# yellow-binary-tree/MMDuet

Measured on AMD Instinct MI355X. Metric: video frames/sec (stream decode, 1fps 336px), higher is better.
Workload: dtype bf16

## Files before the change

mmduet_amd/csrc/gemm.hip:

```cpp
#include "common.h"
#include <type_traits>

#include "gemm_ring.h"

template <typename T> struct Frag;
template <> struct Frag<bf16_t> { using type = bf16x8_t; static constexpr int KSTEP = 32; };
template <> struct Frag<float> { using type = float; static constexpr int KSTEP = 4; };

template <typename T, int BM, int BN> struct TileCfg {
    static constexpr int BK = 32;
    static constexpr int PAD = sizeof(T) == 2 ? 8 : 1;
    static constexpr int LD = BK + PAD;
    static constexpr int WM = BM / 2, WN = BN / 2;
    static constexpr int TM = WM / 16, TN = WN / 16;
};

template <typename T, int ROWS, int LD>
__device__ __forceinline__ void stage_tile(T* __restrict__ lds, const T* __restrict__ g, long long ld, int r0, int nrows, int k0, int kend,
                                           int vec, int tid) {
    if constexpr (sizeof(T) == 2) {
        for (int i = tid; i < ROWS * 4; i += 256) {
            int r = i >> 2, c = (i & 3) * 8;
            s16x8_t v = {0, 0, 0, 0, 0, 0, 0, 0};
            int gr = r0 + r, gk = k0 + c;
// ... 96 lines not shown
        __syncthreads();
        if constexpr (sizeof(T) == 2) {
            bf16x8_t xf[C::TM], wf[C::TN];
#pragma unroll
            for (int i = 0; i < C::TM; ++i) xf[i] = *reinterpret_cast<const bf16x8_t*>(Xs + (wm + i * 16 + lr) * C::LD + lq * 8);
#pragma unroll
            for (int j = 0; j < C::TN; ++j) wf[j] = *reinterpret_cast<const bf16x8_t*>(Ws + (wn + j * 16 + lr) * C::LD + lq * 8);
#pragma unroll
            for (int i = 0; i < C::TM; ++i)
#pragma unroll
                for (int j = 0; j < C::TN; ++j) acc[i][j] = __builtin_amdgcn_mfma_f32_16x16x32_bf16(wf[j], xf[i], acc[i][j], 0, 0, 0);
        } else {
#pragma unroll
            for (int kk = 0; kk < C::BK; kk += 4) {
                float xf[C::TM], wf[C::TN];
#pragma unroll
                for (int i = 0; i < C::TM; ++i) xf[i] = Xs[(wm + i * 16 + lr) * C::LD + kk + lq];
#pragma unroll
                for (int j = 0; j < C::TN; ++j) wf[j] = Ws[(wn + j * 16 + lr) * C::LD + kk + lq];
#pragma unroll
                for (int i = 0; i < C::TM; ++i)
#pragma unroll
                    for (int j = 0; j < C::TN; ++j) acc[i][j] = __builtin_amdgcn_mfma_f32_16x16x4f32(wf[j], xf[i], acc[i][j], 0, 0, 0);
            }
        }
    }

    if (gridDim.z > 1) {
        float* ws = p.ws + (long long)blockIdx.z * p.M * p.N;
#pragma unroll
        for (int i = 0; i < C::TM; ++i)
#pragma unroll
            for (int j = 0; j < C::TN; ++j) {
                int m = m0 + wm + i * 16 + lr, n = n0 + wn + j * 16 + lq * 4;
                if (m < p.M) {
                    float* y = ws + (long long)m * p.N + n;
                    if (n + 3 < p.N && (p.N & 3) == 0) *reinterpret_cast<f32x4_t*>(y) = acc[i][j];
                    else for (int r = 0; r < 4; ++r) if (n + r < p.N) y[r] = acc[i][j][r];
                }
            }
        return;
    }
#pragma unroll
    for (int i = 0; i < C::TM; ++i) {
        int m = m0 + wm + i * 16 + lr;
        if (p.epi == EPI_SWIGLU) {
#pragma unroll
            for (int j = 0; j < C::TN; j += 2) {
                int n = n0 + wn + j * 16 + lq * 4;
                float g[4] = {acc[i][j][0], acc[i][j][1], acc[i][j][2], acc[i][j][3]};
                float u[4] = {acc[i][j + 1][0], acc[i][j + 1][1], acc[i][j + 1][2], acc[i][j + 1][3]};
                store4_swiglu<T>(p, m, n, g, u);
            }
        } else {
#pragma unroll
            for (int j = 0; j < C::TN; ++j) {
                int n = n0 + wn + j * 16 + lq * 4;
                float v[4] = {acc[i][j][0], acc[i][j][1], acc[i][j][2], acc[i][j][3]};
                store4<T>(p, m, n, v);
            }
        }
    }
}

template <typename T>
__global__ void splitk_reduce_kernel(GemmP p, int splits) {
    long long idx = (long long)blockIdx.x * blockDim.x + threadIdx.x;
    int n4 = (p.N + 3) / 4;
    if (idx >= (long long)p.M * n4) return;
    int m = (int)(idx / n4), n = (int)(idx % n4) * 4;
    if (p.epi == EPI_SWIGLU) {
        if ((n & 16) != 0) return;
        float g[4] = {0, 0, 0, 0}, u[4] = {0, 0, 0, 0};
        for (int s = 0; s < splits; ++s) {
            const float* w = p.ws + ((long long)s * p.M + m) * p.N + n;
            for (int r = 0; r < 4; ++r) { if (n + r < p.N) g[r] += w[r]; if (n + 16 + r < p.N) u[r] += w[16 + r]; }
        }
        store4_swiglu<T>(p, m, n, g, u);
        return;
    }
    float v[4] = {0, 0, 0, 0};
    for (int s = 0; s < splits; ++s) {
        const float* w = p.ws + ((long long)s * p.M + m) * p.N + n;
        for (int r = 0; r < 4; ++r) if (n + r < p.N) v[r] += w[r];
    }
    store4<T>(p, m, n, v);
}

__global__ void pack_w16x32_kernel(const bf16_t* __restrict__ W, long long ldw, int N, int K, bf16_t* __restrict__ out) {
    long long i = (long long)blockIdx.x * blockDim.x + threadIdx.x;
    int KT = K >> 5;
    long long pieces = (long long)(N >> 4) * KT * 64;
    if (i >= pieces) return;
    int lane = (int)(i & 63);
    long long tile = i >> 6;
    int kt = (int)(tile % KT);
    long long nt = tile / KT;
    const bf16_t* src = W + (nt * 16 + (lane & 15)) * ldw + kt * 32 + (lane >> 4) * 8;
    *reinterpret_cast<s16x8_t*>(out + i * 8) = *reinterpret_cast<const s16x8_t*>(src);
}

hipError_t launch_pack_w(const void* W, int64_t ldw, int N, int K, void* out, hipStream_t st) {
    long long pieces = (long long)(N >> 4) * (K >> 5) * 64;
    if (pieces <= 0) return hipSuccess;
    hipLaunchKernelGGL(pack_w16x32_kernel, dim3(cdiv(pieces, 256)), dim3(256), 0, st, (const bf16_t*)W, (long long)ldw, N, K, (bf16_t*)out);
    return hipGetLastError();
}

__global__ __launch_bounds__(256) void quantize_fp8_rows_kernel(bf16_t* __restrict__ W, int K, uint8_t* __restrict__ q8, float* __restrict__ scale) {
    __shared__ float red[4];
    const long long row = blockIdx.x;
    bf16_t* w = W + row * K;
    float amax = 0.f;
    for (int k = threadIdx.x; k < K; k += 256) amax = fmaxf(amax, fabsf(bf2f(w[k])));
    amax = wave_max(amax);
    if ((threadIdx.x & 63) == 0) red[threadIdx.x >> 6] = amax;
    __syncthreads();
    amax = fmaxf(fmaxf(red[0], red[1]), fmaxf(red[2], red[3]));
    const float sc = amax > 0.f ? amax / 448.0f : 1.0f;
    if (threadIdx.x == 0) scale[row] = sc;
    for (int k = threadIdx.x * 2; k < K; k += 512) {
        const float a = bf2f(w[k]) / sc, b = bf2f(w[k + 1]) / sc;
        const int pk = __builtin_amdgcn_cvt_pk_fp8_f32(a, b, 0, false);
        q8[row * K + k] = (uint8_t)(pk & 0xff); q8[row * K + k + 1] = (uint8_t)((pk >> 8) & 0xff);
        const auto back = __builtin_amdgcn_cvt_pk_f32_fp8(pk, false);
        w[k] = f2bf(back[0]); w[k + 1] = f2bf(back[1]);
    }
}
hipError_t launch_quantize_fp8_rows(void* W, int N, int K, uint8_t* q8, float* scale, hipStream_t st) {
    if (N <= 0 || (K & 1)) return N <= 0 ? hipSuccess : hipErrorInvalidValue;
    hipLaunchKernelGGL(quantize_fp8_rows_kernel, dim3(N), dim3(256), 0, st, (bf16_t*)W, K, q8, scale);
    return hipGetLastError();
}
__global__ void pack_w8_kernel(const uint8_t* __restrict__ q8, int N, int K, uint8_t* __restrict__ out) {
    long long i = (long long)blockIdx.x * blockDim.x + threadIdx.x;
    const int KP = K >> 6;
    const long long pieces = (long long)(N >> 4) * KP * 64;
    if (i >= pieces) return;
    const int lane = (int)(i & 63);
    const long long blk = i >> 6;
    const int kp = (int)(blk % KP);
    const long long nt = blk / KP;
    const uint8_t* src = q8 + (nt * 16 + (lane & 15)) * (long long)K + kp * 64 + (lane >> 4) * 8;
    uint2 lo = *reinterpret_cast<const uint2*>(src), hi = *reinterpret_cast<const uint2*>(src + 32);
    *reinterpret_cast<uint4*>(out + i * 16) = uint4{lo.x, lo.y, hi.x, hi.y};
}
hipError_t launch_pack_w8(const uint8_t* q8, int N, int K, void* out, hipStream_t st) {
    const long long pieces = (long long)(N >> 4) * (K >> 6) * 64;
    if (pieces <= 0) return hipSuccess;
    hipLaunchKernelGGL(pack_w8_kernel, dim3(cdiv(pieces, 256)), dim3(256), 0, st, q8, N, K, (uint8_t*)out);
    return hipGetLastError();
}
__device__ __forceinline__ bf16x8_t fp8x8_to_bf16(unsigned lo, unsigned hi) {
    typedef __attribute__((ext_vector_type(2))) __bf16 b2;
    const b2 a = __builtin_amdgcn_cvt_scalef32_pk_bf16_fp8((int)lo, 1.0f, false), b = __builtin_amdgcn_cvt_scalef32_pk_bf16_fp8((int)lo, 1.0f, true);
    const b2 c = __builtin_amdgcn_cvt_scalef32_pk_bf16_fp8((int)hi, 1.0f, false), d = __builtin_amdgcn_cvt_scalef32_pk_bf16_fp8((int)hi, 1.0f, true);
    return bf16x8_t{a[0], a[1], b[0], b[1], c[0], c[1], d[0], d[1]};
}

__device__ __forceinline__ int xs_slot(int ktl, int kq, int r) { return kq * 16 + (r ^ (kq + 4 * (ktl & 1))); }

template <int MT, int NT, bool W8 = false>
__global__ __launch_bounds__(256) void gemm_skinny_kernel(GemmP p, int KT, int kt_per_split) {
    constexpr int KS = 4;
    __shared__ __attribute__((aligned(16))) bf16_t Xs[2][MT * KS * 64 * 8];
    const int tid = threadIdx.x, lane = tid & 63, wave = tid >> 6;
    const int lr = lane & 15, lq = lane >> 4;
    const int ntiles = p.N >> 4;
    const int nt0 = (blockIdx.x * 4 + wave) * NT;
    const int kt_beg = blockIdx.y * kt_per_split;
    const int kt_end = min(KT, kt_beg + kt_per_split);
    const bf16_t* X = (const bf16_t*)p.X;
    const bf16_t* Wp = (const bf16_t*)p.W;

    f32x4_t acc[MT][NT];
#pragma unroll
    for (int i = 0; i < MT; ++i)
#pragma unroll
        for (int j = 0; j < NT; ++j) acc[i][j] = f32x4_t{0, 0, 0, 0};

    bf16x8_t wc[NT][KS], wn[NT][KS];
    s16x8_t xr[MT];

    auto load_w = [&](bf16x8_t (&w)[NT][KS], int kt) {
        if constexpr (W8) {
            const uint8_t* W8p = (const uint8_t*)p.W;
#pragma unroll
            for (int j = 0; j < NT; ++j)
#pragma unroll
                for (int s = 0; s < KS; s += 2) {
                    u32x4_t v = {0, 0, 0, 0};
                    if (nt0 + j < ntiles && kt + s < kt_end)
                        v = __builtin_nontemporal_load(reinterpret_cast<const u32x4_t*>(W8p + (((long long)(nt0 + j) * (KT >> 1) + ((kt + s) >> 1)) * 64 + lane) * 16));
                    w[j][s] = fp8x8_to_bf16(v[0], v[1]); w[j][s + 1] = fp8x8_to_bf16(v[2], v[3]);
                }
            return;
        }
#pragma unroll
        for (int j = 0; j < NT; ++j)
#pragma unroll
            for (int s = 0; s < KS; ++s) {
                s16x8_t v = {0, 0, 0, 0, 0, 0, 0, 0};
                if (nt0 + j < ntiles && kt + s < kt_end)
                    v = __builtin_nontemporal_load(reinterpret_cast<const s16x8_t*>(Wp + (((long long)(nt0 + j) * KT + kt + s) * 64 + lane) * 8));
                w[j][s] = __builtin_bit_cast(bf16x8_t, v);
            }
    };
    auto load_x = [&](int kt) {
#pragma unroll
        for (int j = 0; j < MT; ++j) {
            int i = tid + 256 * j, m = i >> 4, c = i & 15;
            s16x8_t v = {0, 0, 0, 0, 0, 0, 0, 0};
            if (m < p.M && kt + (c >> 2) < kt_end) v = *reinterpret_cast<const s16x8_t*>(X + (long long)m * p.ldx + kt * 32 + c * 8);
            xr[j] = v;
        }
    };
    auto write_x = [&](int buf) {
#pragma unroll
        for (int j = 0; j < MT; ++j) {
            int i = tid + 256 * j, m = i >> 4, c = i & 15;
            int mt = m >> 4, r = m & 15, ktl = c >> 2, kq = c & 3;
            *reinterpret_cast<s16x8_t*>(&Xs[buf][((mt * KS + ktl) * 64 + xs_slot(ktl, kq, r)) * 8]) = xr[j];
        }
    };

    load_w(wc, kt_beg);
    load_x(kt_beg);
    write_x(0);
    __syncthreads();
    int cur = 0;
    for (int kt = kt_beg; kt < kt_end; kt += KS) {
        const bool more = kt + KS < kt_end;
        if (more) { load_w(wn, kt + KS); load_x(kt + KS); }
#pragma unroll
        for (int s = 0; s < KS; ++s) {
            if (kt + s < kt_end) {
#pragma unroll
                for (int i = 0; i < MT; ++i) {
                    bf16x8_t xf = *reinterpret_cast<const bf16x8_t*>(&Xs[cur][((i * KS + s) * 64 + xs_slot(s, lq, lr)) * 8]);
#pragma unroll
                    for (int j = 0; j < NT; ++j) acc[i][j] = __builtin_amdgcn_mfma_f32_16x16x32_bf16(wc[j][s], xf, acc[i][j], 0, 0, 0);
                }
            }
        }
        if (more) write_x(cur ^ 1);
        __syncthreads();
#pragma unroll
        for (int j = 0; j < NT; ++j)
#pragma unroll
            for (int s = 0; s < KS; ++s) wc[j][s] = wn[j][s];
        cur ^= 1;
    }

    if (gridDim.y > 1 || p.slabs) {
        float* ws = p.ws + (long long)blockIdx.y * p.M * p.N;
#pragma unroll
        for (int i = 0; i < MT; ++i)
#pragma unroll
            for (int j = 0; j < NT; ++j) {
                int m = i * 16 + lr, n = (nt0 + j) * 16 + lq * 4;
                if (m < p.M && nt0 + j < ntiles) {
                    f32x4_t v = acc[i][j];
                    if (p.slabs && p.wscale) v *= *reinterpret_cast<const f32x4_t*>(p.wscale + n);
                    *reinterpret_cast<f32x4_t*>(ws + (long long)m * p.N + n) = v;
                }
            }
        return;
    }
#pragma unroll
    for (int i = 0; i < MT; ++i) {
        int m = i * 16 + lr;
        if (p.epi == EPI_SWIGLU) {
            if constexpr (NT >= 2) {
#pragma unroll
                for (int j = 0; j < NT; j += 2) {
                    if (nt0 + j + 1 < ntiles) {
                        int n = (nt0 + j) * 16 + lq * 4;
                        float g[4] = {acc[i][j][0], acc[i][j][1], acc[i][j][2], acc[i][j][3]};
                        float u[4] = {acc[i][j + 1][0], acc[i][j + 1][1], acc[i][j + 1][2], acc[i][j + 1][3]};
                        store4_swiglu<bf16_t>(p, m, n, g, u);
                    }
                }
            }
        } else {
#pragma unroll
            for (int j = 0; j < NT; ++j) {
                if (nt0 + j < ntiles) {
                    int n = (nt0 + j) * 16 + lq * 4;
                    float v[4] = {acc[i][j][0], acc[i][j][1], acc[i][j][2], acc[i][j][3]};
                    store4<bf16_t>(p, m, n, v);
                }
            }
        }
    }
}

__device__ __forceinline__ s16x8_t chain_norm8(const s16x8_t& h, const s16x8_t& g, float inv) {
    s16x8_t o;
#pragma unroll
    for (int e = 0; e < 8; ++e) o[e] = (short)f2bf(bf2f((bf16_t)g[e]) * bf2f(f2bf(bf2f((bf16_t)h[e]) * inv)));
    return o;
}

template <int NT, int U, bool W8 = false, bool CHAIN = false, int WAVES = 4>
__global__ __launch_bounds__(WAVES * 64) void gemm_gemv16_kernel(GemmP p, int KT, GemvChain ch) {
    __shared__ __attribute__((aligned(16))) float red[WAVES - 1][NT][64][4];
    constexpr int XW = 1024;
    __shared__ __attribute__((aligned(16))) bf16_t xs[(CHAIN && WAVES == 4) ? WAVES * GEMV_CHAIN_ROWS * XW : 8];
    const int tid = threadIdx.x, lane = tid & 63, wave = tid >> 6;
    const int lr = lane & 15, lq = lane >> 4;
    const int nt0 = blockIdx.x * NT;
    constexpr int KG = W8 ? 2 : 1;
    const int KTg = KT / KG;
    const int ktb = (KTg + gridDim.y - 1) / gridDim.y;
    const int blk_beg = blockIdx.y * ktb, blk_end = min(KTg, blk_beg + ktb);
    const int ktw = (blk_end - blk_beg + WAVES - 1) / WAVES;
    const int kt_beg = blk_beg + wave * ktw, kt_end = min(blk_end, kt_beg + ktw);
    const bool xn = CHAIN && WAVES == 4 && ch.xn_h != nullptr;
    const bf16_t* xrow = (const bf16_t*)p.X + (long long)lr * p.ldx + lq * 8;
    const bf16_t* xl = xs + (wave * GEMV_CHAIN_ROWS + lr) * XW + lq * 8 - kt_beg * (32 * KG);
    const bool row_ok = lr < p.M;

    f32x4_t acc[NT];
#pragma unroll
    for (int j = 0; j < NT; ++j) acc[j] = f32x4_t{0, 0, 0, 0};

    auto chain_prologue = [&]() {
        const int k0 = kt_beg * (32 * KG), kn = (kt_end - kt_beg) * (32 * KG);
        for (int r = 0; r < p.M; ++r) {
            const f32x4_t q = *reinterpret_cast<const f32x4_t*>(ch.xn_ssq + r * GEMV_SSQ_STRIDE + lane * 4);
            s16x8_t hv[2], gv[2];
#pragma unroll
            for (int ps = 0; ps < 2; ++ps) {
                const int k = ps * 512 + lane * 8;
                hv[ps] = s16x8_t{0, 0, 0, 0, 0, 0, 0, 0}; gv[ps] = hv[ps];
                if (k < kn) {
                    hv[ps] = *reinterpret_cast<const s16x8_t*>((const bf16_t*)ch.xn_h + (long long)r * p.K + k0 + k);
                    gv[ps] = *reinterpret_cast<const s16x8_t*>((const bf16_t*)ch.xn_gamma + k0 + k);
                }
            }
            const float inv = rsqrtf(wave_sum((q[0] + q[1]) + (q[2] + q[3])) / (float)p.K + ch.xn_eps);
#pragma unroll
            for (int ps = 0; ps < 2; ++ps) {
                const int k = ps * 512 + lane * 8;
                if (k < kn) *reinterpret_cast<s16x8_t*>(xs + (wave * GEMV_CHAIN_ROWS + r) * XW + k) = chain_norm8(hv[ps], gv[ps], inv);
            }
        }
    };

    if constexpr (W8) {
        const uint8_t* W8p = (const uint8_t*)p.W;
        const int KP = KT >> 1;
        constexpr int UP = U / 2;
        auto iter = [&](int kp0, auto first) {
            u32x4_t wv[NT][UP]; bf16x8_t x[UP][2];
#pragma unroll
            for (int u = 0; u < UP; ++u) {
                const int kp = kp0 + u;
                s16x8_t x0 = {0, 0, 0, 0, 0, 0, 0, 0}, x1 = x0;
                if (kp < kt_end) {
#pragma unroll
                    for (int j = 0; j < NT; ++j)
                        wv[j][u] = __builtin_nontemporal_load(reinterpret_cast<const u32x4_t*>(W8p + (((long long)(nt0 + j) * KP + kp) * 64 + lane) * 16));
                    if (!xn && row_ok) { x0 = *reinterpret_cast<const s16x8_t*>(xrow + kp * 64); x1 = *reinterpret_cast<const s16x8_t*>(xrow + kp * 64 + 32); }
                } else {
#pragma unroll
                    for (int j = 0; j < NT; ++j) wv[j][u] = u32x4_t{0, 0, 0, 0};
                }
                x[u][0] = __builtin_bit_cast(bf16x8_t, x0); x[u][1] = __builtin_bit_cast(bf16x8_t, x1);
            }
            if constexpr (CHAIN) if (xn) {
                if constexpr (decltype(first)::value) chain_prologue();
#pragma unroll
                for (int u = 0; u < UP; ++u) if (row_ok && kp0 + u < kt_end) {
                    x[u][0] = __builtin_bit_cast(bf16x8_t, *reinterpret_cast<const s16x8_t*>(xl + (kp0 + u) * 64));
                    x[u][1] = __builtin_bit_cast(bf16x8_t, *reinterpret_cast<const s16x8_t*>(xl + (kp0 + u) * 64 + 32));
                }
            }
#pragma unroll
            for (int u = 0; u < UP; ++u)
#pragma unroll
                for (int j = 0; j < NT; ++j) {
                    acc[j] = __builtin_amdgcn_mfma_f32_16x16x32_bf16(fp8x8_to_bf16(wv[j][u][0], wv[j][u][1]), x[u][0], acc[j], 0, 0, 0);
                    acc[j] = __builtin_amdgcn_mfma_f32_16x16x32_bf16(fp8x8_to_bf16(wv[j][u][2], wv[j][u][3]), x[u][1], acc[j], 0, 0, 0);
                }
        };
        if (kt_beg < kt_end) {
            iter(kt_beg, std::true_type{});
            for (int kp0 = kt_beg + UP; kp0 < kt_end; kp0 += UP) iter(kp0, std::false_type{});
        }
    } else {
        const bf16_t* Wp = (const bf16_t*)p.W;
        auto iter = [&](int kt0, auto first) {
            bf16x8_t w[NT][U], x[U];
#pragma unroll
            for (int u = 0; u < U; ++u) {
                const int kt = kt0 + u;
                s16x8_t xv = {0, 0, 0, 0, 0, 0, 0, 0};
                if (kt < kt_end) {
#pragma unroll
                    for (int j = 0; j < NT; ++j)
                        w[j][u] = __builtin_bit_cast(bf16x8_t, __builtin_nontemporal_load(reinterpret_cast<const s16x8_t*>(Wp + (((long long)(nt0 + j) * KT + kt) * 64 + lane) * 8)));
                    if (!xn && row_ok) xv = *reinterpret_cast<const s16x8_t*>(xrow + kt * 32);
                } else {
#pragma unroll
                    for (int j = 0; j < NT; ++j) w[j][u] = __builtin_bit_cast(bf16x8_t, xv);
                }
                x[u] = __builtin_bit_cast(bf16x8_t, xv);
            }
            if constexpr (CHAIN) if (xn) {
                if constexpr (decltype(first)::value) chain_prologue();
#pragma unroll
                for (int u = 0; u < U; ++u) if (row_ok && kt0 + u < kt_end) x[u] = __builtin_bit_cast(bf16x8_t, *reinterpret_cast<const s16x8_t*>(xl + (kt0 + u) * 32));
            }
#pragma unroll
            for (int u = 0; u < U; ++u)
#pragma unroll
                for (int j = 0; j < NT; ++j) acc[j] = __builtin_amdgcn_mfma_f32_16x16x32_bf16(w[j][u], x[u], acc[j], 0, 0, 0);
        };
        if (kt_beg < kt_end) {
            iter(kt_beg, std::true_type{});
            for (int kt0 = kt_beg + U; kt0 < kt_end; kt0 += U) iter(kt0, std::false_type{});
        }
    }
    if (wave > 0) {
#pragma unroll
        for (int j = 0; j < NT; ++j) *reinterpret_cast<f32x4_t*>(&red[wave - 1][j][lane][0]) = acc[j];
    }
    __syncthreads();
    if (wave != 0) return;
#pragma unroll
    for (int j = 0; j < NT; ++j)
#pragma unroll
        for (int w2 = 0; w2 < WAVES - 1; ++w2) acc[j] += *reinterpret_cast<const f32x4_t*>(&red[w2][j][lane][0]);
    const int m = lr;
    if constexpr (CHAIN) if (ch.fin_h) {
#pragma unroll
        for (int j = 0; j < NT; ++j) {
            float ss = 0.f;
            if (m < p.M) {
                f32x4_t v = acc[j];
                if (p.wscale) v *= *reinterpret_cast<const f32x4_t*>(p.wscale + (nt0 + j) * 16 + lq * 4);
                bf16_t* hp = (bf16_t*)ch.fin_h + (long long)m * p.N + (nt0 + j) * 16 + lq * 4;
                const s16x4_t r = *reinterpret_cast<const s16x4_t*>(hp);
                s16x4_t o;
#pragma unroll
                for (int e = 0; e < 4; ++e) {
                    const float hv = bf2f(f2bf(bf2f(f2bf(v[e])) + bf2f((bf16_t)r[e])));
                    ss += hv * hv; o[e] = (short)f2bf(hv);
                }
                *reinterpret_cast<s16x4_t*>(hp) = o;
            }
            ss += __shfl_xor(ss, 16, 64); ss += __shfl_xor(ss, 32, 64);
            if (lq == 0 && m < p.M) ch.fin_ssq[m * GEMV_SSQ_STRIDE + nt0 + j] = ss;
        }
        return;
    }
    if (m >= p.M) return;
    if (p.slabs) {
        float* ws = p.ws + (long long)blockIdx.y * p.M * p.N;
#pragma unroll
        for (int j = 0; j < NT; ++j) {
            f32x4_t v = acc[j];
            if (p.wscale) v *= *reinterpret_cast<const f32x4_t*>(p.wscale + (nt0 + j) * 16 + lq * 4);
            *reinterpret_cast<f32x4_t*>(ws + (long long)m * p.N + (nt0 + j) * 16 + lq * 4) = v;
        }
        return;
    }
    if (p.epi == EPI_SWIGLU) {
        if constexpr (NT >= 2) {
#pragma unroll
            for (int j = 0; j < NT; j += 2) {
                float g[4] = {acc[j][0], acc[j][1], acc[j][2], acc[j][3]};
                float u[4] = {acc[j + 1][0], acc[j + 1][1], acc[j + 1][2], acc[j + 1][3]};
                store4_swiglu<bf16_t>(p, m, (nt0 + j) * 16 + lq * 4, g, u);
            }
        }
    } else {
#pragma unroll
        for (int j = 0; j < NT; ++j) {
            float v[4] = {acc[j][0], acc[j][1], acc[j][2], acc[j][3]};
            store4<bf16_t>(p, m, (nt0 + j) * 16 + lq * 4, v);
        }
    }
}

template <int N_, typename F> __device__ __forceinline__ void stream_static_for(F&& f) {
    if constexpr (N_ > 0) { stream_static_for<N_ - 1>(f); f(std::integral_constant<int, N_ - 1>{}); }
}

template <int MT, int NT, int WK, int KS, int NB, int DBG = 0, int WN = 4>
__global__ __launch_bounds__(64 * WN * WK) void gemm_stream_kernel(GemmP p, int KT, int kt_per_block) {
    constexpr int NWAVE = WN * WK, KSB = WK * KS;
    constexpr int XPIECES = MT * KSB;
    constexpr int XP = DBG == 1 ? 0 : (XPIECES + NWAVE - 1) / NWAVE;
    constexpr int NWL = DBG == 2 ? 0 : NT * KS;
    constexpr int LA = NB - 1;
    constexpr int ISSUE = NWL + XP;
    constexpr int VM_STEP = (LA - 1) * ISSUE;
    constexpr int XSLOT = XPIECES * 512;
    static_assert(VM_STEP <= 63, "vmcnt is a 6-bit counter");
    extern __shared__ __attribute__((aligned(16))) bf16_t lds[];
    const int tid = threadIdx.x, lane = tid & 63, wave = __builtin_amdgcn_readfirstlane(tid >> 6);
    const int lr = lane & 15, lq = lane >> 4;
    const int wn = wave % WN, wk = wave / WN;
    const int ntiles = p.N >> 4;
    const int nt0 = (blockIdx.x * WN + wn) * NT;
    const int kt_beg = blockIdx.y * kt_per_block;
    const int kt_end = min(KT, kt_beg + kt_per_block);
    const int nsteps = (kt_end - kt_beg) / KSB;
    const bf16_t* X = (const bf16_t*)p.X;
    const bf16_t* Wp = (const bf16_t*)p.W;

    const int srow = lane >> 2, spos = lane & 3;
    const int sswz = (0x1230 >> (((srow >> 2) & 3) * 4)) & 3;
    unsigned xo[XP + 1];
#pragma unroll
    for (int j = 0; j < XP; ++j) {
        const int pi = (wave + NWAVE * j) % XPIECES;
        int row = (pi / KSB) * 16 + srow; row = row < p.M ? row : p.M - 1;
        xo[j] = (unsigned)(row * (int)p.ldx + (pi % KSB) * 32 + ((spos ^ sswz) * 8)) * 2u;
    }
    long long wo[NT];
#pragma unroll
    for (int j = 0; j < NT; ++j) { int nt = nt0 + j; nt = nt < ntiles ? nt : ntiles - 1; wo[j] = ((long long)nt * KT + kt_beg + wk * KS) * 1024; }
    const unsigned wlane = lane * 16;
    auto dma_x = [&](int slot, int step, int j) {
        const char* ub = (const char*)X + ((long long)kt_beg + (long long)step * KSB) * 64;
        __builtin_amdgcn_global_load_lds((const __attribute__((address_space(1))) void*)(ub + xo[j]),
                                         (__attribute__((address_space(3))) void*)(lds + slot * XSLOT + ((wave + NWAVE * j) % XPIECES) * 512), 16, 0, 0);
    };
    auto load_w = [&](bf16x8_t& dst, int j, int ks, int step) {
        const unsigned long long ua = (unsigned long long)(uintptr_t)((const char*)Wp + wo[j] + ((long long)step * KSB + ks) * 1024);
        const unsigned long long ub = ((unsigned long long)(unsigned)__builtin_amdgcn_readfirstlane((unsigned)(ua >> 32)) << 32) |
                                      (unsigned long long)(unsigned)__builtin_amdgcn_readfirstlane((unsigned)ua);
        asm volatile("global_load_dwordx4 %0, %1, %2 nt" : "=v"(dst) : "v"(wlane), "s"(ub) : "memory");
    };
    const int rswz = (0x1230 >> (((lr >> 2) & 3) * 4)) & 3;
    const int aoff = lr * 32 + ((lq ^ rswz) * 8);

    f32x4_t acc[MT][NT];
#pragma unroll
    for (int i = 0; i < MT; ++i)
#pragma unroll
        for (int j = 0; j < NT; ++j) acc[i][j] = f32x4_t{0, 0, 0, 0};
    bf16x8_t wb[NB][NT][KS];

    auto issue = [&](int step, auto buf_c) {
        constexpr int buf = decltype(buf_c)::value;
        if constexpr (DBG != 2) {
#pragma unroll
            for (int j = 0; j < NT; ++j)
#pragma unroll
                for (int ks = 0; ks < KS; ++ks) load_w(wb[buf][j][ks], j, ks, step);
        }
#pragma unroll
        for (int j = 0; j < XP; ++j) dma_x(buf, step, j);
    };
    stream_static_for<LA>([&](auto uc) { constexpr int u = decltype(uc)::value; if (u < nsteps) issue(u, std::integral_constant<int, u>{}); });

    auto step = [&](int s, auto buf_c, bool steady) {
        constexpr int cur = decltype(buf_c)::value, nxt = (cur + LA) % NB;
        if (steady) asm volatile("s_waitcnt vmcnt(%0)" :: "i"(VM_STEP) : "memory");
        else asm volatile("s_waitcnt vmcnt(0)" ::: "memory");
        MMD_BAR();
        __builtin_amdgcn_sched_barrier(0);
        if (s + LA < nsteps) issue(s + LA, std::integral_constant<int, nxt>{});
        __builtin_amdgcn_sched_barrier(0);
        const bf16_t* xs = lds + cur * XSLOT;
#pragma unroll
        for (int ks = 0; ks < KS; ++ks) {
            const int ktl = wk * KS + ks;
#pragma unroll
            for (int i = 0; i < MT; ++i) {
                if constexpr (DBG == 1) {
#pragma unroll
                    for (int j = 0; j < NT; ++j) if (i == 0) { const u32x4_t w4 = __builtin_bit_cast(u32x4_t, wb[cur][j][ks]); asm volatile("" :: "v"(w4[0]), "v"(w4[1]), "v"(w4[2]), "v"(w4[3])); }
                    continue;
                }
                const bf16x8_t xf = *reinterpret_cast<const bf16x8_t*>(xs + (i * KSB + ktl) * 512 + aoff);
#pragma unroll
                for (int j = 0; j < NT; ++j) acc[i][j] = __builtin_amdgcn_mfma_f32_16x16x32_bf16(wb[cur][j][ks], xf, acc[i][j], 0, 0, 0);
            }
        }
    };
    int s = 0;
    for (; s + NB + LA <= nsteps; s += NB)
        stream_static_for<NB>([&](auto uc) { constexpr int u = decltype(uc)::value; step(s + u, std::integral_constant<int, u>{}, true); });
    for (; s < nsteps; )
        stream_static_for<NB>([&](auto uc) { constexpr int u = decltype(uc)::value; if (s < nsteps) { step(s, std::integral_constant<int, u>{}, s + LA < nsteps); ++s; } });

    if constexpr (WK > 1) {
        __syncthreads();
        float* red = reinterpret_cast<float*>(lds);
        if (wk > 0) {
#pragma unroll
            for (int i = 0; i < MT; ++i)
#pragma unroll
                for (int j = 0; j < NT; ++j) *reinterpret_cast<f32x4_t*>(red + ((((wk - 1) * WN + wn) * MT + i) * NT + j) * 256 + lane * 4) = acc[i][j];
        }
        __syncthreads();
        if (wk > 0) return;
#pragma unroll
        for (int w2 = 0; w2 < WK - 1; ++w2)
#pragma unroll
            for (int i = 0; i < MT; ++i)
#pragma unroll
                for (int j = 0; j < NT; ++j) acc[i][j] += *reinterpret_cast<const f32x4_t*>(red + (((w2 * WN + wn) * MT + i) * NT + j) * 256 + lane * 4);
    }
    if (gridDim.y > 1 || p.slabs) {
        float* ws = p.ws + (long long)blockIdx.y * p.M * p.N;
#pragma unroll
        for (int i = 0; i < MT; ++i)
#pragma unroll
            for (int j = 0; j < NT; ++j) {
                const int m = i * 16 + lr, n = (nt0 + j) * 16 + lq * 4;
                if (m < p.M && nt0 + j < ntiles) {
                    f32x4_t v = acc[i][j];
                    if (p.slabs && p.wscale) v *= *reinterpret_cast<const f32x4_t*>(p.wscale + n);
                    *reinterpret_cast<f32x4_t*>(ws + (long long)m * p.N + n) = v;
                }
            }
        return;
    }
    if (p.epi == EPI_SWIGLU) {
        if constexpr (NT >= 2) {
            stream_static_for<MT>([&](auto ic) {
                constexpr int i = decltype(ic)::value;
                const int m = i * 16 + lr;
#pragma unroll
                for (int j = 0; j < NT; j += 2) {
                    if (m < p.M && nt0 + j + 1 < ntiles) {
                        const int n_gate = (nt0 + j) * 16 + lq * 4;
                        *reinterpret_cast<s16x4_t*>((bf16_t*)p.Y + (long long)m * p.ldy + (n_gate >> 5) * 16 + (n_gate & 15)) = big_value_swiglu(acc[i][j], acc[i][j + 1], p.wscale, n_gate);
                    }
                }
            });
        }
        return;
    }
    stream_static_for<MT>([&](auto ic) {
        constexpr int i = decltype(ic)::value;
        const int m = i * 16 + lr;
#pragma unroll
        for (int j = 0; j < NT; ++j) {
            if (nt0 + j < ntiles) {
                float v[4] = {acc[i][j][0], acc[i][j][1], acc[i][j][2], acc[i][j][3]};
                store4<bf16_t>(p, m, (nt0 + j) * 16 + lq * 4, v);
            }
        }
    });
}

static void launch_reduce(void (*kernel)(GemmP, int), const GemmP& p, int splits, hipStream_t st) {
    long long work = (long long)p.M * ((p.N + 3) / 4);
    hipLaunchKernelGGL(kernel, dim3(cdiv(work, 256)), dim3(256), 0, st, p, splits);
}
static void launch_gemv16(const GemmP& p, const GemmPlan& pl, const GemvChain* chain, hipStream_t st) {
    const int KT = p.K >> 5;
    const GemvChain none;
    const GemvChain& ch = pl.chain != GEMV_PLAIN ? *chain : none;
    const bool w8 = pl.w_from == GEMM_W_PACKED8, two = pl.nt == 2, chained = pl.chain != GEMV_PLAIN;
    if (pl.chain == GEMV_PRODUCER) {
        GemmP q = p; q.slabs = 0;
        if (w8) hipLaunchKernelGGL((gemm_gemv16_kernel<1, 8, true, true, 16>), dim3(pl.gx), dim3(1024), 0, st, q, KT, ch);
        else hipLaunchKernelGGL((gemm_gemv16_kernel<1, 8, false, true, 16>), dim3(pl.gx), dim3(1024), 0, st, q, KT, ch);
        return;
    }
    const dim3 grid(pl.gx, pl.splits);
#define GEMV16_GO(NT_, W8_, CH_) hipLaunchKernelGGL((gemm_gemv16_kernel<NT_, 8, W8_, CH_>), grid, dim3(256), 0, st, p, KT, ch)
    if (w8) { if (two) { if (chained) GEMV16_GO(2, true, true); else GEMV16_GO(2, true, false); } else { if (chained) GEMV16_GO(1, true, true); else GEMV16_GO(1, true, false); } }
    else    { if (two) { if (chained) GEMV16_GO(2, false, true); else GEMV16_GO(2, false, false); } else { if (chained) GEMV16_GO(1, false, true); else GEMV16_GO(1, false, false); } }
#undef GEMV16_GO
}

template <int MT, int NT, int WK, int KS, int NB, int DBG = 0, int WN = 4>
static void launch_stream_t(const GemmP& p, const GemmPlan& pl, hipStream_t st) {
    constexpr int KSB = WK * KS;
    constexpr size_t ring = (size_t)NB * MT * KSB * 1024, red = (size_t)(WK - 1) * WN * MT * NT * 1024;
    constexpr size_t smem = ring > red ? ring : red;
    static bool attr_set[64] = {};
    int adev = 0; hipGetDevice(&adev);
    if (smem > 65536 && adev >= 0 && adev < 64 && !attr_set[adev]) {
        hipFuncSetAttribute((const void*)gemm_stream_kernel<MT, NT, WK, KS, NB, DBG, WN>, hipFuncAttributeMaxDynamicSharedMemorySize, (int)smem);
        attr_set[adev] = true;
    }
    hipLaunchKernelGGL((gemm_stream_kernel<MT, NT, WK, KS, NB, DBG, WN>), dim3(pl.gx, pl.splits), dim3(64 * WN * WK), smem, st, p, p.K >> 5, pl.kt_per_block);
    if (pl.reduce) launch_reduce(splitk_reduce_kernel<bf16_t>, p, pl.splits, st);
}
template <int MT, int NT, int WK, int KS, int NB>
static void launch_stream_wn(const GemmP& p, const GemmPlan& pl, hipStream_t st) {
    switch (pl.wn) {
        case 5: return launch_stream_t<MT, NT, WK, KS, NB, 0, 5>(p, pl, st);
        case 6: return launch_stream_t<MT, NT, WK, KS, NB, 0, 6>(p, pl, st);
        case 7: return launch_stream_t<MT, NT, WK, KS, NB, 0, 7>(p, pl, st);
        case 8: return launch_stream_t<MT, NT, WK, KS, NB, 0, 8>(p, pl, st);
        default: return launch_stream_t<MT, NT, WK, KS, NB, 0, 4>(p, pl, st);
    }
}
static void launch_stream(const GemmP& p, const GemmPlan& pl, hipStream_t st) {
    const bool two = pl.nt == 2;
    if (pl.mt == 4) return two ? launch_stream_wn<4, 2, 1, 4, 3>(p, pl, st) : launch_stream_wn<4, 1, 1, 4, 3>(p, pl, st);
    if (pl.mt == 8) return two ? launch_stream_wn<8, 2, 1, 2, 4>(p, pl, st) : launch_stream_wn<8, 1, 1, 4, 3>(p, pl, st);
    return two ? launch_stream_wn<16, 2, 1, 1, 4>(p, pl, st) : launch_stream_wn<16, 1, 1, 2, 4>(p, pl, st);
}

template <int MT>
static void launch_skinny_mt(const GemmP& p, const GemmPlan& pl, hipStream_t st) {
    const int KT = p.K >> 5;
    const dim3 grid(pl.gx, pl.splits);
    if (pl.w_from == GEMM_W_PACKED8) {
        if (pl.nt == 2) hipLaunchKernelGGL((gemm_skinny_kernel<MT, 2, true>), grid, dim3(256), 0, st, p, KT, pl.kt_per_block);
        else hipLaunchKernelGGL((gemm_skinny_kernel<MT, 1, true>), grid, dim3(256), 0, st, p, KT, pl.kt_per_block);
    } else if (pl.nt == 2) hipLaunchKernelGGL((gemm_skinny_kernel<MT, 2>), grid, dim3(256), 0, st, p, KT, pl.kt_per_block);
    else hipLaunchKernelGGL((gemm_skinny_kernel<MT, 1>), grid, dim3(256), 0, st, p, KT, pl.kt_per_block);
    if (pl.reduce) launch_reduce(splitk_reduce_kernel<bf16_t>, p, pl.splits, st);
}

template <int BN, int EPI, bool F16 = false, int BM = 128>
__global__ __launch_bounds__(256) void gemm_big_kernel(GemmP p, int KT) {
    constexpr int BK = 64;
    static_assert(BM % 32 == 0, "two wave rows of whole 16-row tiles");
    constexpr int TM = BM / 32, TN = BN / 32;
    constexpr int XE = BM * BK, WE = BN * BK;
    __shared__ __attribute__((aligned(16))) bf16_t lds[2 * (XE + WE)];
    const int tid = threadIdx.x, lane = tid & 63, wave = tid >> 6;
    const int lr = lane & 15, lq = lane >> 4;
    const int wm = (wave >> 1) * (BM / 2), wn = (wave & 1) * (BN / 2);
    const int nbx = gridDim.x, nby = gridDim.y;
    int bid = blockIdx.y * nbx + blockIdx.x;
    const int nblk = nbx * nby;
    {
        const int xcd = bid & 7, q = nblk >> 3, r = nblk & 7;
        bid = (xcd < r ? xcd * (q + 1) : r * (q + 1) + (xcd - r) * q) + (bid >> 3);
    }
    int mt, nt;
    if (p.N > p.M) { nt = bid / nby; mt = bid % nby; } else { mt = bid / nbx; nt = bid % nbx; }
    const int m0 = mt * BM, n0 = nt * BN;
    const bf16_t* X = (const bf16_t*)p.X;
    const bf16_t* Wp = (const bf16_t*)p.W;
    const int nsteps = p.K / BK;

    auto stage = [&](int buf, int step) {
        bf16_t* xs = lds + buf * (XE + WE);
        bf16_t* ws = xs + XE;
        const int k0 = step * BK;
#pragma unroll
// ... 285 lines not shown
```

Measured before the change: 361.7.

## Software-pipeline decode GEMV loads with buffer resources and overlap chain prologue

```diff
diff --git a/mmduet_amd/csrc/gemm.hip b/mmduet_amd/csrc/gemm.hip
--- a/mmduet_amd/csrc/gemm.hip
+++ b/mmduet_amd/csrc/gemm.hip
@@ -422,12 +422,19 @@
     return o;
 }
 
+constexpr unsigned GEMV_OOB = 0x80000000u;
+__device__ __forceinline__ __amdgpu_buffer_rsrc_t gemv_rsrc(const void* base, int bytes) {
+    return __builtin_amdgcn_make_buffer_rsrc(const_cast<void*>(base), 0, bytes, 0x00020000);
+}
+__device__ __forceinline__ u32x4_t gemv_ld16(__amdgpu_buffer_rsrc_t r, unsigned off) { return __builtin_bit_cast(u32x4_t, __builtin_amdgcn_raw_buffer_load_b128(r, off, 0, 0)); }
+__device__ __forceinline__ u32x4_t gemv_ld16_nt(__amdgpu_buffer_rsrc_t r, unsigned off) { return __builtin_bit_cast(u32x4_t, __builtin_amdgcn_raw_buffer_load_b128(r, off, 0, 2)); }
+
 template <int NT, int U, bool W8 = false, bool CHAIN = false, int WAVES = 4>
 __global__ __launch_bounds__(WAVES * 64) void gemm_gemv16_kernel(GemmP p, int KT, GemvChain ch) {
     __shared__ __attribute__((aligned(16))) float red[WAVES - 1][NT][64][4];
     constexpr int XW = 1024;
     __shared__ __attribute__((aligned(16))) bf16_t xs[(CHAIN && WAVES == 4) ? WAVES * GEMV_CHAIN_ROWS * XW : 8];
-    const int tid = threadIdx.x, lane = tid & 63, wave = tid >> 6;
+    const int tid = threadIdx.x, lane = tid & 63, wave = __builtin_amdgcn_readfirstlane(tid >> 6);
     const int lr = lane & 15, lq = lane >> 4;
     const int nt0 = blockIdx.x * NT;
     constexpr int KG = W8 ? 2 : 1;
@@ -436,112 +443,96 @@
     const int blk_beg = blockIdx.y * ktb, blk_end = min(KTg, blk_beg + ktb);
     const int ktw = (blk_end - blk_beg + WAVES - 1) / WAVES;
     const int kt_beg = blk_beg + wave * ktw, kt_end = min(blk_end, kt_beg + ktw);
-    const bool xn = CHAIN && WAVES == 4 && ch.xn_h != nullptr;
-    const bf16_t* xrow = (const bf16_t*)p.X + (long long)lr * p.ldx + lq * 8;
-    const bf16_t* xl = xs + (wave * GEMV_CHAIN_ROWS + lr) * XW + lq * 8 - kt_beg * (32 * KG);
+    constexpr bool XN = CHAIN && WAVES == 4;
     const bool row_ok = lr < p.M;
+    const bf16_t* xl = xs + (wave * GEMV_CHAIN_ROWS + (row_ok ? lr : 0)) * XW + lq * 8 - kt_beg * (32 * KG);
+    constexpr int D = ((WAVES == 4 && NT == 1) ? 2 * U : U) / KG;
 
     f32x4_t acc[NT];
 #pragma unroll
     for (int j = 0; j < NT; ++j) acc[j] = f32x4_t{0, 0, 0, 0};
 
-    auto chain_prologue = [&]() {
-        const int k0 = kt_beg * (32 * KG), kn = (kt_end - kt_beg) * (32 * KG);
-        for (int r = 0; r < p.M; ++r) {
-            const f32x4_t q = *reinterpret_cast<const f32x4_t*>(ch.xn_ssq + r * GEMV_SSQ_STRIDE + lane * 4);
-            s16x8_t hv[2], gv[2];
+    s16x4_t fin_r = {0, 0, 0, 0};
+    if constexpr (CHAIN && WAVES != 4) if (ch.fin_h && wave == 0 && row_ok) fin_r = *reinterpret_cast<const s16x4_t*>((const bf16_t*)ch.fin_h + (long long)lr * p.N + nt0 * 16 + lq * 4);
+
+    if (kt_beg < kt_end) {
+        __amdgpu_buffer_rsrc_t wr[NT];
+#pragma unroll
+        for (int j = 0; j < NT; ++j) wr[j] = gemv_rsrc((const char*)p.W + (long long)(nt0 + j) * KTg * 1024, kt_end * 1024);
+        const __amdgpu_buffer_rsrc_t xr = gemv_rsrc(p.X, (int)(((long long)(p.M - 1) * p.ldx + p.K) * 2));
+        const unsigned x_lane = row_ok ? (unsigned)((lr * p.ldx + lq * 8) * 2) : GEMV_OOB;
+        u32x4_t w[NT][D], xg[XN ? 1 : D][KG];
+        auto issue = [&](int u, int kt) {
+#pragma unroll
+            for (int j = 0; j < NT; ++j) w[j][u] = gemv_ld16_nt(wr[j], (unsigned)(kt * 1024 + lane * 16));
+            if constexpr (!XN) {
+#pragma unroll
+                for (int g = 0; g < KG; ++g) xg[u][g] = gemv_ld16(xr, kt < kt_end ? x_lane + (unsigned)((kt * KG + g) * 64) : GEMV_OOB);
+            }
+        };
+        auto consume = [&](int u, int kt) {
+            if (kt < kt_end) {
+                bf16x8_t xf[KG];
+#pragma unroll
+                for (int g = 0; g < KG; ++g) {
+                    if constexpr (XN) {
+                        const s16x8_t v = *reinterpret_cast<const s16x8_t*>(xl + (kt * KG + g) * 32);
+                        xf[g] = __builtin_bit_cast(bf16x8_t, row_ok ? v : s16x8_t{0, 0, 0, 0, 0, 0, 0, 0});
+                    } else xf[g] = __builtin_bit_cast(bf16x8_t, xg[u][g]);
+                }
+#pragma unroll
+                for (int j = 0; j < NT; ++j) {
+                    if constexpr (W8) {
+                        acc[j] = __builtin_amdgcn_mfma_f32_16x16x32_bf16(fp8x8_to_bf16(w[j][u][0], w[j][u][1]), xf[0], acc[j], 0, 0, 0);
+                        acc[j] = __builtin_amdgcn_mfma_f32_16x16x32_bf16(fp8x8_to_bf16(w[j][u][2], w[j][u][3]), xf[KG - 1], acc[j], 0, 0, 0);
+                    } else acc[j] = __builtin_amdgcn_mfma_f32_16x16x32_bf16(__builtin_bit_cast(bf16x8_t, w[j][u]), xf[0], acc[j], 0, 0, 0);
+                }
+            }
+        };
+
+#pragma unroll
+        for (int u = 0; u < D / 2; ++u) issue(u, kt_beg + u);
+        u32x4_t pq[GEMV_CHAIN_ROWS], ph[GEMV_CHAIN_ROWS][2], pg[2];
+        const int kn = (kt_end - kt_beg) * (32 * KG);
+        if constexpr (XN) {
+            __builtin_amdgcn_sched_barrier(0);
+            const int k0 = kt_beg * (32 * KG);
+            const __amdgpu_buffer_rsrc_t sr = gemv_rsrc(ch.xn_ssq, p.M * GEMV_SSQ_STRIDE * 4), hr = gemv_rsrc(ch.xn_h, p.M * p.K * 2), gr = gemv_rsrc(ch.xn_gamma, p.K * 2);
+#pragma unroll
+            for (int r = 0; r < GEMV_CHAIN_ROWS; ++r) pq[r] = gemv_ld16(sr, (unsigned)((r * GEMV_SSQ_STRIDE + lane * 4) * 4));
 #pragma unroll
             for (int ps = 0; ps < 2; ++ps) {
                 const int k = ps * 512 + lane * 8;
-                hv[ps] = s16x8_t{0, 0, 0, 0, 0, 0, 0, 0}; gv[ps] = hv[ps];
-                if (k < kn) {
-                    hv[ps] = *reinterpret_cast<const s16x8_t*>((const bf16_t*)ch.xn_h + (long long)r * p.K + k0 + k);
-                    gv[ps] = *reinterpret_cast<const s16x8_t*>((const bf16_t*)ch.xn_gamma + k0 + k);
-                }
-            }
-            const float inv = rsqrtf(wave_sum((q[0] + q[1]) + (q[2] + q[3])) / (float)p.K + ch.xn_eps);
-#pragma unroll
-            for (int ps = 0; ps < 2; ++ps) {
-                const int k = ps * 512 + lane * 8;
-                if (k < kn) *reinterpret_cast<s16x8_t*>(xs + (wave * GEMV_CHAIN_ROWS + r) * XW + k) = chain_norm8(hv[ps], gv[ps], inv);
-            }
-        }
-    };
-
-    if constexpr (W8) {
-        const uint8_t* W8p = (const uint8_t*)p.W;
-        const int KP = KT >> 1;
-        constexpr int UP = U / 2;
-        auto iter = [&](int kp0, auto first) {
-            u32x4_t wv[NT][UP]; bf16x8_t x[UP][2];
-#pragma unroll
-            for (int u = 0; u < UP; ++u) {
-                const int kp = kp0 + u;
-                s16x8_t x0 = {0, 0, 0, 0, 0, 0, 0, 0}, x1 = x0;
-                if (kp < kt_end) {
-#pragma unroll
-                    for (int j = 0; j < NT; ++j)
-                        wv[j][u] = __builtin_nontemporal_load(reinterpret_cast<const u32x4_t*>(W8p + (((long long)(nt0 + j) * KP + kp) * 64 + lane) * 16));
-                    if (!xn && row_ok) { x0 = *reinterpret_cast<const s16x8_t*>(xrow + kp * 64); x1 = *reinterpret_cast<const s16x8_t*>(xrow + kp * 64 + 32); }
-                } else {
-#pragma unroll
-                    for (int j = 0; j < NT; ++j) wv[j][u] = u32x4_t{0, 0, 0, 0};
-                }
-                x[u][0] = __builtin_bit_cast(bf16x8_t, x0); x[u][1] = __builtin_bit_cast(bf16x8_t, x1);
-            }
-            if constexpr (CHAIN) if (xn) {
-                if constexpr (decltype(first)::value) chain_prologue();
-#pragma unroll
-                for (int u = 0; u < UP; ++u) if (row_ok && kp0 + u < kt_end) {
-                    x[u][0] = __builtin_bit_cast(bf16x8_t, *reinterpret_cast<const s16x8_t*>(xl + (kp0 + u) * 64));
-                    x[u][1] = __builtin_bit_cast(bf16x8_t, *reinterpret_cast<const s16x8_t*>(xl + (kp0 + u) * 64 + 32));
-                }
-            }
-#pragma unroll
-            for (int u = 0; u < UP; ++u)
-#pragma unroll
-                for (int j = 0; j < NT; ++j) {
-                    acc[j] = __builtin_amdgcn_mfma_f32_16x16x32_bf16(fp8x8_to_bf16(wv[j][u][0], wv[j][u][1]), x[u][0], acc[j], 0, 0, 0);
-                    acc[j] = __builtin_amdgcn_mfma_f32_16x16x32_bf16(fp8x8_to_bf16(wv[j][u][2], wv[j][u][3]), x[u][1], acc[j], 0, 0, 0);
-                }
-        };
-        if (kt_beg < kt_end) {
-            iter(kt_beg, std::true_type{});
-            for (int kp0 = kt_beg + UP; kp0 < kt_end; kp0 += UP) iter(kp0, std::false_type{});
-        }
-    } else {
-        const bf16_t* Wp = (const bf16_t*)p.W;
-        auto iter = [&](int kt0, auto first) {
-            bf16x8_t w[NT][U], x[U];
-#pragma unroll
-            for (int u = 0; u < U; ++u) {
-                const int kt = kt0 + u;
-                s16x8_t xv = {0, 0, 0, 0, 0, 0, 0, 0};
-                if (kt < kt_end) {
-#pragma unroll
-                    for (int j = 0; j < NT; ++j)
-                        w[j][u] = __builtin_bit_cast(bf16x8_t, __builtin_nontemporal_load(reinterpret_cast<const s16x8_t*>(Wp + (((long long)(nt0 + j) * KT + kt) * 64 + lane) * 8)));
-                    if (!xn && row_ok) xv = *reinterpret_cast<const s16x8_t*>(xrow + kt * 32);
-                } else {
-#pragma unroll
-                    for (int j = 0; j < NT; ++j) w[j][u] = __builtin_bit_cast(bf16x8_t, xv);
-                }
-                x[u] = __builtin_bit_cast(bf16x8_t, xv);
-            }
-            if constexpr (CHAIN) if (xn) {
-                if constexpr (decltype(first)::value) chain_prologue();
-#pragma unroll
-                for (int u = 0; u < U; ++u) if (row_ok && kt0 + u < kt_end) x[u] = __builtin_bit_cast(bf16x8_t, *reinterpret_cast<const s16x8_t*>(xl + (kt0 + u) * 32));
-            }
-#pragma unroll
-            for (int u = 0; u < U; ++u)
-#pragma unroll
-                for (int j = 0; j < NT; ++j) acc[j] = __builtin_amdgcn_mfma_f32_16x16x32_bf16(w[j][u], x[u], acc[j], 0, 0, 0);
-        };
-        if (kt_beg < kt_end) {
-            iter(kt_beg, std::true_type{});
-            for (int kt0 = kt_beg + U; kt0 < kt_end; kt0 += U) iter(kt0, std::false_type{});
-        }
+                pg[ps] = gemv_ld16(gr, k < kn ? (unsigned)((k0 + k) * 2) : GEMV_OOB);
+#pragma unroll
+                for (int r = 0; r < GEMV_CHAIN_ROWS; ++r) ph[r][ps] = gemv_ld16(hr, k < kn ? (unsigned)((r * p.K + k0 + k) * 2) : GEMV_OOB);
+            }
+            __builtin_amdgcn_sched_barrier(0);
+        }
+#pragma unroll
+        for (int u = D / 2; u < D; ++u) issue(u, kt_beg + u);
+        if constexpr (XN) {
+            __builtin_amdgcn_sched_barrier(0);
+#pragma unroll
+            for (int r = 0; r < GEMV_CHAIN_ROWS; ++r) {
+                if (r < p.M) {
+                    const f32x4_t q = __builtin_bit_cast(f32x4_t, pq[r]);
+                    const float inv = rsqrtf(wave_sum((q[0] + q[1]) + (q[2] + q[3])) / (float)p.K + ch.xn_eps);
+#pragma unroll
+                    for (int ps = 0; ps < 2; ++ps) {
+                        const int k = ps * 512 + lane * 8;
+                        if (k < kn) *reinterpret_cast<s16x8_t*>(xs + (wave * GEMV_CHAIN_ROWS + r) * XW + k) = chain_norm8(__builtin_bit_cast(s16x8_t, ph[r][ps]), __builtin_bit_cast(s16x8_t, pg[ps]), inv);
+                    }
+                }
+            }
+        }
+        int kt0 = kt_beg;
+        for (; kt0 + D < kt_end; kt0 += D) {
+#pragma unroll
+            for (int u = 0; u < D; ++u) { consume(u, kt0 + u); issue(u, kt0 + D + u); }
+        }
+#pragma unroll
+        for (int u = 0; u < D; ++u) consume(u, kt0 + u);
     }
     if (wave > 0) {
 #pragma unroll
@@ -562,7 +553,7 @@
                 f32x4_t v = acc[j];
                 if (p.wscale) v *= *reinterpret_cast<const f32x4_t*>(p.wscale + (nt0 + j) * 16 + lq * 4);
                 bf16_t* hp = (bf16_t*)ch.fin_h + (long long)m * p.N + (nt0 + j) * 16 + lq * 4;
-                const s16x4_t r = *reinterpret_cast<const s16x4_t*>(hp);
+                const s16x4_t r = fin_r;
                 s16x4_t o;
 #pragma unroll
                 for (int e = 0; e < 4; ++e) {
```

After: 359.8. No clear change (-0.5%).
